# giech/usrp_nfc

Measured on AMD Instinct MI355X. Metric: IQ Msamples/s -> decoded bits (2 Msps stream), higher is better.
Workload: dtype f32 envelope / f64 window sums / u8 symbols; 1 GPU; configs[1]: Miller-only decode, synthetic IQ @2 Msps; input_kind=fc32 IQ, 8 B/sample (envelope computed in the kernel), samples_per_gpu=100000000, parallelism=time-chunk x1, edges_per_gpu=6627699, symbols_reader=3971547, symbols_tag=0, packets=101186, boundary_redos=0, exchange=none, stepping=sync, in_flight=1

## Files before the change

### usrp_nfc_amd/csrc/host_context.h

```cpp
#pragma once


namespace {

std::string g_create_error;

}

enum : int {
    TOT_RUNS = 0,
    TOT_EDGES = 8,
    TOT_DECMAP = 16,
    TOT_SPEC = 40,
    TOT_PKT0 = 72,
    TOT_PKT1 = 80,
    TOT_LAST2 = 88,
    TOT_NSYM = 96,
    TOT_CERT = 104,
    TOT_FRAME = 128,
    TOT_BYTES = 160
};

static_assert(sizeof(CertSummary) <= TOT_FRAME - TOT_CERT, "the verdict summary fits its slot of the totals");
struct DevState {
// ... 1 lines not shown
    EdgeCarry ecarry;
    DecCarry dcarry;
    uint8_t totals[TOT_BYTES];
    uint32_t seq[4];
};

constexpr size_t AHEAD_LDS_MAX = 96 * 1024;
constexpr int LEAN_STEPS_AHEAD = 4;
constexpr int NRING = 4;
constexpr int NSUB = 3;

namespace {
struct Switches {
    std::optional<std::string> debug_clk;
    std::optional<int> no_small, debug_bad_launch, debug_redo_submitted, debug, trace, trace_alloc, no_submit_ahead, wg, wg_rounds, wg_bulk, wg_rerun, wg_rowbal, wg_nr, wg_per_cu, wg_per_cu_ahead, wg_ex, lean, lean_rounds,
        lean_waves, edge_prefix, dec_spec, dec_runin, spin_wait, chunk_adapt, chunk_mult;
    std::optional<double> lean_gfac, lean_gmin, eps;
    std::optional<unsigned long> own_prefix_max;
    std::optional<std::pair<int, int>> wg_lone;
    std::optional<std::array<double, 3>> rowbal_f;
    std::optional<bool> ring_global;
};
inline Switches read_switches() {
    Switches s;
#ifdef NFC_TEST_HOOKS
    const struct { const char *name; std::optional<int> Switches::*at; } ints[] = {
        {"NFC_NO_SMALL", &Switches::no_small}, {"NFC_DEBUG_BAD_LAUNCH", &Switches::debug_bad_launch}, {"NFC_DEBUG_REDO_SUBMITTED", &Switches::debug_redo_submitted},
        {"NFC_DEBUG", &Switches::debug}, {"NFC_TRACE", &Switches::trace}, {"NFC_TRACE_ALLOC", &Switches::trace_alloc}, {"NFC_NO_SUBMIT_AHEAD", &Switches::no_submit_ahead},
        {"NFC_WG", &Switches::wg}, {"NFC_WG_ROUNDS", &Switches::wg_rounds}, {"NFC_WG_BULK", &Switches::wg_bulk},
        {"NFC_WG_RERUN", &Switches::wg_rerun}, {"NFC_WG_NR", &Switches::wg_nr}, {"NFC_WG_PER_CU", &Switches::wg_per_cu},
        {"NFC_WG_PER_CU_AHEAD", &Switches::wg_per_cu_ahead}, {"NFC_WG_EX", &Switches::wg_ex}, {"NFC_LEAN", &Switches::lean}, {"NFC_LEAN_ROUNDS", &Switches::lean_rounds},
        {"NFC_LEAN_WAVES", &Switches::lean_waves}, {"NFC_EDGE_PREFIX", &Switches::edge_prefix}, {"NFC_DEC_SPEC", &Switches::dec_spec}, {"NFC_DEC_RUNIN", &Switches::dec_runin},
        {"NFC_SPIN_WAIT", &Switches::spin_wait}, {"NFC_CHUNK_ADAPT", &Switches::chunk_adapt}, {"NFC_CHUNK_MULT", &Switches::chunk_mult}};
    const struct { const char *name; std::optional<double> Switches::*at; } reals[] = {
        {"NFC_LEAN_GFAC", &Switches::lean_gfac}, {"NFC_LEAN_GMIN", &Switches::lean_gmin}, {"NFC_EPS", &Switches::eps}};
    for (const auto &v : ints)
        if (const char *e = getenv(v.name)) s.*v.at = atoi(e);
    for (const auto &v : reals)
        if (const char *e = getenv(v.name)) s.*v.at = atof(e);
    if (const char *e = getenv("NFC_DEBUG_CLK")) s.debug_clk = e;
    if (const char *e = getenv("NFC_OWN_PREFIX_MAX")) s.own_prefix_max = strtoul(e, nullptr, 10);
    if (const char *e = getenv("NFC_WG_LONE")) {
        int a = 4, b = 64;
        if (sscanf(e, "%d,%d", &a, &b) >= 1) s.wg_lone = std::make_pair(a, b);
    }
    if (const char *e = getenv("NFC_WG_ROWBAL")) {
        std::array<double, 3> f{0.0, 1.0, 1.0};
        if (sscanf(e, "%lf,%lf,%lf", &f[0], &f[1], &f[2]) >= 2 && f[0] > 0.5 && f[0] < 1.5 && f[1] > 0.5 && f[1] < 1.5 && f[2] > 0.5 && f[2] < 1.5)
// ... 48 lines not shown
    float eps;
    float i16_scale;
    size_t in_bytes_per_sample;
    hipStream_t st = nullptr;
    Stream own_st;
    Stream st_a;
    Event ev[8];
    DevBuf d_gring;
    bool state_dirty = false, dirty_fill_ring = false;
    float dirty_fill = 0.f;
    Carry dirty_carry;
    EdgeCarry dirty_ecarry;
    DecCarry dirty_dcarry;
    bool cert_pending = false;
    CertLaunch cert;
    bool dbg_bad_launch = false, dbg_redo_submitted = false, dbg_no_submit_ahead = false, dbg_any = false, dbg_clk = false, dbg_trace = false;
    std::string dbg_clk_path;
    uint32_t batch_seq = 0;
    int timing = 0;
    Event kev[2 * 6];
    int n_kev = 0;
    std::string err;
    LaunchError launch_err;

    DevBuf d_mil_map, d_man_map, d_mil_out, d_man_out, d_qmil_map, d_qmil_step;
    uint8_t mil_q_of[16], mil_canon[16];
    DecTables T;

    DevBuf d_state, d_ring[NRING];
    PinBuf hs_pin{hipHostMallocMapped | hipHostMallocCoherent};
// ... 156 lines not shown
    LaunchError &le = launch_error();
    if (le.err != hipSuccess) {
        const LaunchError e = le;
        le = LaunchError{};
        return fail(c, NFC_ERR_DEVICE, "kernel launch failed: %s (%s:%d)", hipGetErrorString(e.err), e.file, e.line);
    }
    if (with_mirror && c->hs->seq[0] != c->batch_seq)
        return fail(c, NFC_ERR_DEVICE, "state mirror is stale (batch %u, mirror %u): a kernel of this batch did not run", c->batch_seq, c->hs->seq[0]);
    return NFC_OK;
}
#define BATCHCHK(c, with_mirror)                                   \
    do {                                                           \
        if (int rc__ = batch_ok((c), (with_mirror))) return rc__;  \
    } while (0)

void launch_fill_kind(nfc_ctx *c, const void *in, uint32_t n, int nchunks, int ring_idx = -1) {
    float *ring = c->d_ring[ring_idx < 0 ? c->ring_cur : ring_idx].as<float>();
    Carry *cr = dC(c);
    EdgeCarryInit eci{(int32_t *)dE(c), c->L % c->mx};
    uint8_t *ver = c->d_ver.as<uint8_t>();
    CertSummary *sum = (CertSummary *)(dT(c) + TOT_CERT);
    StateInit init;
    memset(&init, 0, sizeof init);
    int fresh = 0;
    if (c->state_dirty) {
        static_assert(offsetof(DevState, totals) <= sizeof init.words && offsetof(DevState, totals) % 4 == 0, "state head fits");
        DevState h;
        h.carry = c->dirty_carry;
        h.ecarry = c->dirty_ecarry;
        h.dcarry = c->dirty_dcarry;
        init.apply = 1;
        init.n_words = (int32_t)(offsetof(DevState, totals) / 4);
        memcpy(init.words, &h, offsetof(DevState, totals));
        init.dst = (uint32_t *)c->d_state.p;
        init.fill_ring = c->dirty_fill_ring ? 1 : 0;
        init.fill = c->dirty_fill;
        init.ring_len = c->Lpad;
        c->state_dirty = c->dirty_fill_ring = false;
        fresh = h.carry.stable == 0 && h.carry.filled == 0 && n >= (uint32_t)c->L && (void *)cr == c->d_state.p;
    }
    NFC_LAUNCH(c->kk->fill, dim3(1), dim3(FILL_BLOCK), (size_t)c->Lpad * 4, c->st, in, n, c->i16_scale, c->L, ring, cr, eci, ver, nchunks, sum, init,
               &((DevState *)c->d_state.p)->seq[0], c->batch_seq, fresh);
}
void launch_seq_kind(nfc_ctx *c, const SeqArgs &A) { NFC_LAUNCH(c->kk->seq, dim3(1), dim3(64), 0, c->st, A); }

int ceil_log2(int v) {
    int b = 0;
    while ((1 << b) < v) b++;
    return b;
}

double elapsed_ms(hipEvent_t a, hipEvent_t b) {
    float ms = 0;
    (void)hipEventElapsedTime(&ms, a, b);
    return ms;
}

// ... 3 lines not shown
```

### usrp_nfc_amd/csrc/host_stages.h

```cpp
#pragma once

namespace {

__global__ __launch_bounds__(256) void k_certify_and_write(CertLaunch C, EdgeArgs E, size_t nwords, const EdgeAgg *partials, const EdgeAgg *supers,
                                                          const EdgeRec *recs, uint32_t *epos, uint16_t *ecode, uint32_t cap, bool own_prefix, uint32_t *total_out,
                                                          Last2 *last2_total, EdgeCarry *carry_out) {
    const uint32_t tiles = gridDim.x - C.blocks;
    if (blockIdx.x == 0) {
        certify_block(C.A, C.cert, nullptr, C.ring_next, C.carry, C.sum, C.blocks - 1, C.blocks);
        return;
    }
    if (blockIdx.x > tiles) {
        certify_block(C.A, C.cert, nullptr, C.ring_next, C.carry, C.sum, blockIdx.x - tiles - 1, C.blocks);
        return;
    }
    write_edges_tile(E, nwords, partials, supers, recs, epos, ecode, cap, own_prefix, total_out, last2_total, carry_out, tiles - blockIdx.x, tiles);
}

int run_edges(nfc_ctx *c, uint32_t n, uint32_t skip, uint64_t g0, bool beside_threshold = false) {
    uint8_t *tot = dT(c);
    const size_t nwords = ((size_t)n + 63) / 64;
    EdgeArgs E;
    E.neg = c->d_neg.as<uint64_t>();
    E.pos = c->d_pos.as<uint64_t>();
    E.n = n;
    E.skip = skip;
    E.mx = c->mx;
    E.dur_in = c->h_ecarry.dur;
    E.last_bit_in = c->h_ecarry.last_bit;
    E.state_in = c->h_ecarry.state;
    E.nd = c->mx + 1;
// ... 3 lines not shown
    for (int b = 0; b < 64; b += c->mx) E.per_mask |= 1ull << b;
    E.sw = (uint32_t)(EW_WORDS * EW_SUPER);
    E.tps = (uint32_t)EW_SUPER;
    const size_t tiles = edge_num_tiles(nwords);
    const size_t supers = edge_num_supers(nwords);
    HIPCHK(c, c->d_partials.ensure((tiles + supers + 2) * sizeof(EdgeAgg)));
    EdgeAgg *parts = c->d_partials.as<EdgeAgg>();
    EdgeAgg *sups = parts + tiles + 1;
    const bool use_recs = c->edge_prefix < 0 ? !beside_threshold : c->edge_prefix != 0;
    if (use_recs) HIPCHK(c, c->d_edge_rec.ensure(std::max<size_t>(tiles, 1) * SCAN_BLOCK * sizeof(EdgeRec)));
    EdgeRec *recs = use_recs ? c->d_edge_rec.as<EdgeRec>() : nullptr;
    const bool own = tiles <= c->own_prefix_max;
    Last2 *last2_total = (Last2 *)(tot + TOT_LAST2);
    uint32_t *edges_total = (uint32_t *)(tot + TOT_EDGES);
    const EdgeAggOp op{E.mx, E.mx_magic};
    if (tiles) NFC_LAUNCH(k_edge_reduce, dim3((unsigned)supers), dim3(ER_BLOCK), 0, c->st, E, nwords, parts, sups, recs);
    if (!own || !tiles)
        scan_partials_with(c->st, op, supers, nullptr, (uint32_t)(EW_WORDS * EW_SUPER), sups, op.identity(), (EdgeAgg *)nullptr,
                           EdgeTotalEpilogue{E, edges_total, last2_total, dE(c)});
    const uint32_t cap = c->cap_edges;
    const size_t cap_al = std::max(cap, c->alloc_edges);
    HIPCHK(c, c->d_epos.ensure((cap_al + 8) * 4));
    HIPCHK(c, c->d_ecode.ensure((cap_al + 8) * 2));
    if (c->cert_pending && tiles) {
        c->cert_pending = false;
        NFC_LAUNCH(k_certify_and_write, dim3((unsigned)(c->cert.blocks + tiles)), dim3(SCAN_BLOCK), 0, c->st, c->cert, E, nwords, parts, sups, recs,
                   c->d_epos.as<uint32_t>(), c->d_ecode.as<uint16_t>(), cap, own, edges_total, last2_total, dE(c));
    } else if (tiles) {
        NFC_LAUNCH(k_write_edges, dim3((unsigned)tiles), dim3(SCAN_BLOCK), 0, c->st, E, nwords, parts, sups, recs, c->d_epos.as<uint32_t>(),
                   c->d_ecode.as<uint16_t>(), cap, own, edges_total, last2_total, dE(c));
    }
// ... 349 lines not shown
            }
            const int r = run_small(c, n, skip, g0);
            if (r) return r;
            if (!ev3_done && c->timing >= 2) HIPCHK(c, hipEventRecord(c->ev[3], c->st));
            ev3_done = true;
            return NFC_OK;
        }
        int r = run_edges(c, n, skip, g0);
        if (r) return r;
        if (!ev3_done && c->timing >= 2) HIPCHK(c, hipEventRecord(c->ev[3], c->st));
        ev3_done = true;
        return run_decode(c);
    };
    const std::function<int()> ahead = edges_and_decode;
    bool clean = false;
    int rc = run_threshold(c, d_in, n, skip, want_edges ? &ahead : nullptr, &clean);
    if (rc) return rc;
    if (want_edges) {
        bool decode_only = false;
        int respeculated = 0;
        for (int attempt = 0;; attempt++) {
            if (attempt > 0 || !clean || decode_only) {
                if (decode_only) {
                    rc = run_decode(c, true);
                } else {
                    rc = edges_and_decode();
                }
                if (rc) return rc;
                HIPCHK(c, hipStreamSynchronize(c->st));
            }
// ... 73 lines not shown
```

### usrp_nfc_amd/csrc/host_threshold.h

```cpp
#pragma once

namespace {

static bool sums_exact(const Carry &hc, int emin, int emax, uint32_t vtop) {
    int low = emin - 23;
    if (hc.ss_emin != 255) low = std::min(low, hc.ss_emin);
    float vtf;
    memcpy(&vtf, &vtop, 4);
    int high = 255 + 64;
    if (std::isfinite(vtf) && vtf >= 0.f) high = vtf > 0.f ? std::ilogb((double)vtf) + 127 : 0;
    high = std::max(high, hc.ss_emax);
    return (emax < 255) && (high - low <= 52);
}

static inline void eps_adapt(nfc_ctx *c, const CertSummary &s) {
    if (!c->dbg_trace) return;
    float w;
    memcpy(&w, &s.worst, 4);
    fprintf(stderr, "[nfc] eps %.5f: the speculation used %.5f of the window sum at most, %u chunks failed their certification\n", (double)c->eps, (double)w, s.n_fail);
}

static inline void cpu_relax() {
#if defined(__x86_64__) || defined(__i386__)
    __builtin_ia32_pause();
// ... 244 lines not shown
    A.nlist = 0;
    A.mode = 0;
    A.cert = P.d_cert;
    A.sum = (CertSummary *)(dT(c) + TOT_CERT);
    A.ksteps = P.form == ThrForm::Workgroup ? c->wg_rounds : c->lean_rounds;
    A.gfac = c->lean_gfac;
    A.gfloor = c->lean_gmin;
    A.blk = 1 << c->nfold;
    launch_threshold(c, P, ThrLaunch::Pass0, A, P.nch, own_events);
}
static void enqueue_certify(nfc_ctx *c, const ThrPlan &P, const ThrArgs &A, CertInfo *info, float *ring_out, CertSummary *sum) {
    NFC_LAUNCH(k_certify, dim3(cert_grid(A.nlist)), dim3(256), 0, c->st, A, P.d_cert, info, ring_out, dC(c), sum);
}

static int threshold_span(nfc_ctx *c, const void *d_in_all, uint32_t n_all, uint32_t skip_all, uint32_t base, const EdgeCarry &ec,
                          const std::function<int()> *ahead, bool *clean, bool *need_seq_out, bool *recut_out = nullptr) {
    bool ran_ahead = false;
    *clean = false;
    const int L = c->L;
    const uint32_t n = n_all - base;
    const uint32_t skip = skip_all > base ? skip_all - base : 0u;
    const void *d_in = (const char *)d_in_all + (size_t)base * c->in_bytes_per_sample;
    const uint64_t nseen = c->nseen + base;
    uint32_t passes = 0;
    ThrArgs A;
    ThrPlan P;
    if (int rc = thr_prepare(c, d_in, n, n_all, skip, base, nseen, ec, c->ring_cur, c->d_neg, c->d_pos, false, A, P)) return rc;
    const uint32_t nch = P.nch;
    const bool wg = P.form == ThrForm::Workgroup;
    uint8_t *d_cert = P.d_cert;
    const uint8_t *h_cert = P.h_cert, *h_gflags = P.h_gflags, *h_gmin = P.h_gmin, *h_gmax = P.h_gmax;

    launch_fill_kind(c, d_in, n, (int)nch);

    const bool force_seq = (c->P.flags & NFC_FLAG_FORCE_SEQUENTIAL) != 0 || L < STEP;
    bool need_seq = force_seq;
    if (!force_seq) {
        const bool lean = wg || P.form == ThrForm::Lean;
        const bool dbg_clk = lean && c->dbg_clk;
        if (dbg_clk) {
            HIPCHK(c, c->d_certinfo.ensure((size_t)nch * 32 * 5));
            A.dbg_clk = c->d_certinfo.as<unsigned long long>();
        }
        enqueue_pass0(c, P, A);
        if (dbg_clk) {
            std::vector<unsigned long long> h((size_t)nch * 4);
            HIPCHK(c, hipStreamSynchronize(c->st));
            HIPCHK(c, hipMemcpy(h.data(), c->d_certinfo.p, (size_t)nch * 32, hipMemcpyDeviceToHost));
            unsigned long long t0 = ~0ull, t1 = 0;
            double pro = 0, loop = 0, epi = 0, maxtot = 0, maxstart = 0;
            for (uint32_t k = 0; k < nch; k++) {
                t0 = std::min(t0, h[4 * k]);
                t1 = std::max(t1, h[4 * k + 3]);
            }
            for (uint32_t k = 0; k < nch; k++) {
                pro += (double)(h[4 * k + 1] - h[4 * k]);
                loop += (double)(h[4 * k + 2] - h[4 * k + 1]);
                epi += (double)(h[4 * k + 3] - h[4 * k + 2]);
                maxtot = std::max(maxtot, (double)(h[4 * k + 3] - h[4 * k]));
// ... 78 lines not shown
                flags_with_verdict = first_round && c->fine_left > 0;
                if (!first_round || flags_with_verdict) {
                    HIPCHK(c, hipMemcpyAsync(c->h_cflags.p, c->d_cflags.p, (size_t)4 * nch, hipMemcpyDeviceToHost, c->st));
                    HIPCHK(c, hipMemcpyAsync(P.h_gvtop, c->d_gvtop.p, (size_t)nch * 4, hipMemcpyDeviceToHost, c->st));
                }
                HIPCHK(c, mirror_async(c));
                if (first_round && ahead) {
                    const int rc = (*ahead)();
                    if (rc) return rc;
                    ran_ahead = true;
                }
            }
            if (stamped_last) HIPCHK(c, wait_for_stamp(c));
            else HIPCHK(c, hipStreamSynchronize(c->st));
            BATCHCHK(c, true);
            std::vector<uint32_t> failing;
            if (first_round) {
                memcpy(&summary, c->hs->totals + TOT_CERT, sizeof summary);
                if (base == 0) eps_adapt(c, summary);
                if (summary.n_fail == 0 && !dbg) {
                    have_summary = true;
                    break;
                }
                if (recut_out && c->fine_adapt && wg && c->fine_left == 0 && !c->P.chunk_samples && c->fine_mult > 1 &&
                    (uint64_t)summary.n_fail * 64u > (uint64_t)nch) {
                    *recut_out = true;
                    A.ver_zero = 0;
                    return NFC_OK;
                }
                if (!flags_with_verdict) HIPCHK(c, hipMemcpy(c->h_cflags.p, c->d_cflags.p, (size_t)4 * nch, hipMemcpyDeviceToHost));
// ... 189 lines not shown
    return NFC_OK;
}

int run_threshold(nfc_ctx *c, const void *d_in, uint32_t n, uint32_t skip, const std::function<int()> *ahead, bool *clean) {
    *clean = false;
    c->stats.threshold_passes = 0;
    c->stats.chunks_rerun = 0;
    c->stats.chunks_rerun_in_place = 0;
    c->stats.used_sequential = 0;
    const uint32_t span = (uint32_t)std::min<uint64_t>(((uint64_t)8 * c->L + STEP - 1) / STEP * STEP, 1u << 30);
    EdgeCarry ec = c->h_ecarry;
    uint32_t base = 0;
    for (int round = 0;; round++) {
        bool need_seq = false, span_clean = false;
        const bool optimistic = base == 0 && !(c->fine_adapt && c->fine_left > 0);
        bool recut = false;
        int rc = threshold_span(c, d_in, n, skip, base, ec, optimistic ? ahead : nullptr, &span_clean, &need_seq, &recut);
        if (rc) return rc;
        if (recut) {
            c->fine_left = 8;
            c->cert_pending = false;
            HIPCHK(c, hipMemsetAsync((char *)dC(c) + offsetof(Carry, fin_valid), 0, sizeof(int32_t), c->st));
            span_clean = false;
            rc = threshold_span(c, d_in, n, skip, base, ec, nullptr, &span_clean, &need_seq, nullptr);
            if (rc) return rc;
        }
        if (!need_seq) {
            *clean = span_clean && base == 0;
            if (c->fine_adapt) {
                if ((uint64_t)c->stats.chunks_rerun * 64u > (uint64_t)c->stats.n_chunks) c->fine_left = 8;
                else if (c->fine_left > 0) c->fine_left--;
            }
            return NFC_OK;
        }
        const bool forced = (c->P.flags & NFC_FLAG_FORCE_SEQUENTIAL) != 0 || c->L < STEP;
// ... 11 lines not shown
```

### usrp_nfc_amd/csrc/nfc_amd.hip

```cpp
#include <hip/hip_runtime.h>
#include <hip/hip_ext.h>

#include <algorithm>
#include <atomic>
#include <chrono>
#include <cmath>
#include <cstdarg>
#include <cstdio>
#include <cstdlib>
#include <cstring>
#include <string>
#include <thread>
#include <array>
#include <functional>
#include <memory>
#include <optional>
#include <vector>

#include "../../include/nfc_amd.h"
#include "launch_check.h"
#include "decode.hip.h"
#include "decoder_tables.h"
#include "edges.hip.h"
#include "scan.hip.h"
// ... 183 lines not shown
    if (c->wg_ex_ok) {
        const void *kx = (const void *)c->kk->wg_ex;
        if (c->wg_ex_lds > 64 * 1024) CRT(hipFuncSetAttribute(kx, hipFuncAttributeMaxDynamicSharedMemorySize, (int)c->wg_ex_lds));
        int fit = 0;
        CRT(hipOccupancyMaxActiveBlocksPerMultiprocessor(&fit, kx, 256, c->wg_ex_lds));
        if (fit < 1) c->wg_ex_ok = 0;
        c->wg_ex_max = prop.multiProcessorCount * std::max(1, std::min(4, fit));
    }
    if (sw.wg_ex) {
        if (*sw.wg_ex <= 0) c->wg_ex_ok = 0;
        else c->wg_ex_max = *sw.wg_ex;
    }
    if (!c->wg_rounds) c->wg_rounds = 8;
    if (sw.chunk_adapt) c->fine_adapt = *sw.chunk_adapt != 0;
    if (sw.chunk_mult) c->fine_mult = std::max(1, std::min(16, *sw.chunk_mult));
    return NFC_OK;
}

int create_resources(nfc_ctx *c) {
    CRT(c->own_st.create());
    c->st = c->own_st;
    for (auto &e : c->ev) CRT(e.create());
    for (auto &e : c->kev) CRT(e.create());
    CRT(c->st_a.create());
    for (int b = 0; b < NSUB; b++) {
        CRT(c->ev_a[b].create(hipEventDisableTiming));
        CRT(c->ev_b[b].create(hipEventDisableTiming));
        CRT(c->kev_sub[b][0].create());
        CRT(c->kev_sub[b][1].create());
        CRT(c->hs_a[b].ensure(sizeof(DevState)));
// ... 1063 lines not shown
#ifdef NFC_TEST_HOOKS
extern "C" float nfc_debug_frames_ms(const nfc_ctx *c) { return c && c->frames_ready ? c->fr_ms : -1.f; }
extern "C" void nfc_debug_live_resources(uint64_t out[4]) {
    for (int k = 0; k < 4; k++) out[k] = nfc::live::count(k).load();
}
extern "C" int nfc_debug_dec_lds(const nfc_ctx *c, int which, uint32_t *dyn_bytes, int *wgs_per_cu) {
    if (!c || which < 0 || which > 2 || !dyn_bytes || !wgs_per_cu) return NFC_ERR_ARG;
    const bool lds = 4 * c->T.nd <= nfc::DEC_LDS_ROWS;
    const void *k = which == 0   ? (const void *)nfc::dec_spec_kernel(lds, c->T)
                    : which == 1 ? (lds ? (const void *)nfc::k_dec_reduce<true> : (const void *)nfc::k_dec_reduce<false>)
                                 : (lds ? (const void *)nfc::k_dec_apply<true> : (const void *)nfc::k_dec_apply<false>);
    *dyn_bytes = (uint32_t)c->dec_lds[which];
    if (hipSetDevice(c->P.device) != hipSuccess) return NFC_ERR_DEVICE;
    return hipOccupancyMaxActiveBlocksPerMultiprocessor(wgs_per_cu, k, nfc::SCAN_BLOCK, c->dec_lds[which]) == hipSuccess ? NFC_OK : NFC_ERR_DEVICE;
}
extern "C" int nfc_debug_dec_shapes(const nfc_ctx *c, uint32_t *out6) {
    if (!c || !out6) return NFC_ERR_ARG;
    out6[0] = (uint32_t)nfc::DEC_TILE;
    out6[1] = c->own_prefix_max;
    out6[2] = nfc::ST_CLOSES;
    out6[3] = (uint32_t)nfc::DEC_LDS_ROWS;
    out6[4] = (uint32_t)(nfc::DEC_RUNIN_MAX * nfc::SCAN_BLOCK);
    out6[5] = c->sym_own ? 1u : 0u;
    return NFC_OK;
}
#endif
```

### usrp_nfc_amd/csrc/threshold.hip.h

```cpp
#pragma once
#include <hip/hip_runtime.h>
#include <stdint.h>

#include <type_traits>

namespace nfc {

constexpr int STEP = 256;
constexpr int LL_NONE = -(1 << 30);
constexpr int MAX_FIX_ITERS = 80;
constexpr float RND_SUM = 2.44140625e-04f;

enum : int { IN_IQ_F32 = 0, IN_ENV_F32 = 1, IN_REAL_F32_SQ = 2, IN_I16_SQ = 3, IN_IQ_I16 = 4, IN_IQ_I8 = 5, IN_IQ_U8 = 6 };

#ifndef NFC_HDR_KERNEL_LINKAGE
#define NFC_HDR_KERNEL_LINKAGE
#endif

struct Carry {
    double ss;
    double delta;
    int32_t filled;
    int32_t stable;
    int32_t ss_emin;
// ... 66 lines not shown
    uint32_t nlist;
    int32_t mode;
    int32_t twords;
    int32_t off;
    int32_t nrows;
    uint8_t *cert;
    CertSummary *sum;
    int32_t ksteps;
    float gfac, gfloor;
    int32_t blk;
    int32_t ver_zero;
    int32_t wg_stage_rounds;
    unsigned long long *dbg_clk;
    uint32_t row_len[4], row_start[4], row_div;
    int C_max;
};
__device__ __forceinline__ void chunk_span(const ThrArgs &A, uint32_t c, uint32_t &m_chunk, uint32_t &len) {
    const uint32_t row = min(c / A.row_div, 3u);
    len = A.row_len[row];
    m_chunk = A.row_start[row] + (c - row * A.row_div) * len;
}

__device__ __forceinline__ int rfl(int v) { return __builtin_amdgcn_readfirstlane(v); }
__device__ __forceinline__ uint32_t rfl(uint32_t v) { return (uint32_t)__builtin_amdgcn_readfirstlane((int)v); }
__device__ __forceinline__ float rfl(float v) { return __int_as_float(__builtin_amdgcn_readfirstlane(__float_as_int(v))); }
__device__ __forceinline__ double rfl(double v) {
    return __hiloint2double(__builtin_amdgcn_readfirstlane(__double2hiint(v)), __builtin_amdgcn_readfirstlane(__double2loint(v)));
}
__device__ __forceinline__ bool uni(bool c) { return __builtin_amdgcn_readfirstlane((int)c) != 0; }
template <int CTRL, int ROWMASK>
// ... 1153 lines not shown
    }
}

struct EdgeCarryInit {
    int32_t *dst;
    int32_t dur0;
};

struct StateInit {
    int32_t apply, fill_ring, ring_len, n_words;
    float fill;
    uint32_t *dst;
    uint32_t words[32];
};

template <int KIND>
__global__ __launch_bounds__(FILL_BLOCK) void k_fill(const void *in, uint32_t n, float i16_scale, int L, float *ring, Carry *carry,
                                                     EdgeCarryInit eci, uint8_t *ver, int nchunks, CertSummary *sum, StateInit init,
                                                     uint32_t *seq_dst, uint32_t seq, int fresh) {
    extern __shared__ __attribute__((aligned(16))) unsigned char smem[];
    __shared__ FillRed red;
    float *lr = (float *)smem;
    const int tid = threadIdx.x;
    if (tid == 0 && seq_dst) *seq_dst = seq;
    if (fresh) {
        static_assert(sizeof(Carry) % 4 == 0 && sizeof(Carry) <= sizeof(init.words), "the carry heads the state block");
        constexpr int CW = (int)(sizeof(Carry) / 4);
        if (tid >= CW && tid < init.n_words) init.dst[tid] = init.words[tid];
        double part = 0;
        uint32_t emin = 255u, emax = 0u;
// ... 7 lines not shown
                if (i >= L) break;
                ring[i] = v[k];
                lr[i] = v[k];
                part += (double)v[k];
                if (v[k] != 0.f) {
                    const uint32_t e = max(f32_expfield(v[k]), 1u);
                    emin = min(emin, e);
                    emax = max(emax, e);
                }
            }
        }
        if (init.fill_ring)
            for (int i = L + tid; i < init.ring_len; i += FILL_BLOCK) ring[i] = 0.f;
        for (int i = tid; i < nchunks; i += FILL_BLOCK) ver[i] = 0;
        fill_reduce(red, part, emin, emax);
        if (tid == 0) {
            const double S = part;
            int lg = 0;
            while ((1 << lg) < L) lg++;
            const bool exact = (emax < 255u) && ((int)emax + 2 + lg - ((int)emin - 23) <= 52);
            double s = S, err = 0;
            if (!exact) {
                s = 0;
                for (int i = 0; i < L; i++) {
                    const double v = (double)lr[i];
                    const double t = s + v;
                    const double bv = t - s;
                    err += fabs((s - (t - bv)) + (v - bv));
                    s = t;
                }
            }
            Carry nc;
            uint32_t cw[CW];
#pragma unroll
            for (int k = 0; k < CW; k++) cw[k] = init.words[k];
            memcpy(&nc, cw, sizeof nc);
            nc.filled = L;
            nc.ss = s;
            nc.stable = 1;
            if (err != 0.0) nc.inexact = 1;
            batch_guard(nc, S, emin, emax);
            *carry = nc;
            eci.dst[0] = 0;
            eci.dst[1] = 0;
            eci.dst[2] = eci.dur0;
            if (sum) *sum = CertSummary{0u, 255u, 0u, 0u, 0u, 0u};
        }
        return;
    }
    if (init.apply) {
        if (tid < init.n_words) init.dst[tid] = init.words[tid];
        if (init.fill_ring)
            for (int i = tid; i < init.ring_len; i += FILL_BLOCK) ring[i] = i < L ? init.fill : 0.f;
        __syncthreads();
    }
    if (carry->stable) {
        prepare_batch(ring, L, carry, ver, nchunks, sum, red);
        return;
    }
    const int filled = carry->filled;
    const int can = min((int)n, L - filled);
    double part = 0;
// ... 38 lines not shown
                const double bv = t - s;
                err += fabs((s - (t - bv)) + (v - bv));
                s = t;
            }
        }
        carry->filled = L;
        carry->ss = s;
        carry->stable = 1;
        if (err != 0.0) carry->inexact = 1;
        eci.dst[0] = 0;
        eci.dst[1] = 0;
        eci.dst[2] = eci.dur0;
    }
    for (int i = tid; i < nchunks; i += FILL_BLOCK) ver[i] = 0;
    prepare_batch_finish(carry, sum, S, emin, emax);
}

NFC_HDR_KERNEL_LINKAGE __global__ __launch_bounds__(FIN_BLOCK) void k_finalize_state(ThrArgs A, float *ring_next, Carry *carry) {
    finalize_state(A, ring_next, carry, nullptr);
}

struct SeqArgs {
    const void *in;
    uint32_t n, skip, g0modL;
    int32_t L, mx;
    double lo, hi, hi_plus;
    float i16_scale;
    float *ring;
    Carry *carry;
    int32_t state, last_bit, dur;
// ... 56 lines not shown
```

### usrp_nfc_amd/csrc/threshold_wg.hip.h

```cpp
#pragma once
#include "edges.hip.h"
#include "threshold_lean.hip.h"

namespace nfc {

constexpr int WG_WAVES = 4;
constexpr int wg_round_samples(int nr) { return 64 * nr * WG_WAVES; }
constexpr int WG_NR_MAX = 8;
#ifndef NFC_WG_FR
#define NFC_WG_FR 8
#endif
constexpr int wg_flush_rounds(int nr) { return nr == 4 ? NFC_WG_FR : NFC_WG_FR / 2; }
constexpr size_t wg_stage_bytes(int nr, int rounds) { return (size_t)rounds * (size_t)(2 * WG_WAVES * 2 * nr * 4); }
struct WgShared {
    uint32_t msk[3][WG_WAVES][4 * WG_NR_MAX + 4];
    uint32_t scr[2][WG_WAVES][8];
    int32_t fin[WG_WAVES][4];
    float4 acc[WG_WAVES][64];
    uint32_t flag[WG_WAVES];
    uint32_t cold[WG_WAVES][8];
    float bc[8];
};
constexpr size_t WG_SHARED_BYTES = (sizeof(WgShared) + 15) & ~(size_t)15;

// ... 150 lines not shown
    const int mx = A.mx;
    uint32_t m_chunk_v, chunk_len_v;
    chunk_span(A, c, m_chunk_v, chunk_len_v);
    const uint32_t m_chunk = rfl(m_chunk_v), chunk_len = rfl(chunk_len_v);
    const uint32_t n1 = min(A.n, m_chunk + chunk_len);
    const uint32_t m_start = max(m_chunk, A.skip);
    constexpr int RB = LeanRaw<KIND>::BYTES;
    const uint32_t wbase0 = m_chunk + STEPN * (uint32_t)wave;
    const char *const in_first = (const char *)A.in + (size_t)wbase0 * RB;
    const uint32_t voff = (uint32_t)lane * (uint32_t)RB;
    bool primed = false;
    if (m_chunk >= m_start && m_chunk + (uint32_t)wg_round_samples(NR) <= n1) {
        wg_load_step<KIND, NR>(voff, in_first);
        primed = true;
    }
    const Carry cr = *A.carry;
    uint64_t *const neg_p = A.neg, *const pos_p = A.pos;
    const uintptr_t plane_of_lane = (lane >= 2 * NR) ? (uintptr_t)pos_p : (uintptr_t)neg_p;
    const int plane_dword = (lane >= 2 * NR) ? lane - 2 * NR : lane;
    const float i16s = A.i16_scale;
    const unsigned long long lane_lt = (1ull << lane) - 1ull;
    int scr_par = 0;
    auto wg_gather = [&](const uint32_t (&v)[8], int k, uint32_t (&out)[WG_WAVES][8]) __attribute__((always_inline)) {
        if (lane == 0)
            for (int i = 0; i < k; i++) sh->scr[scr_par][wave][i] = v[i];
        wg_barrier();
        for (int w = 0; w < WG_WAVES; w++)
            for (int i = 0; i < k; i++) out[w][i] = rfl(sh->scr[scr_par][w][i]);
        scr_par ^= 1;
    };

// ... 20 lines not shown
#ifdef NFC_WG_PROF
    unsigned long long pf_take = 0, pf_b1 = 0, pf_b2 = 0, pf_rounds = 0, pf_t = 0;
#define WG_PF_BEGIN() pf_t = clock64()
#define WG_PF_END(acc) acc += clock64() - pf_t
#else
#define WG_PF_BEGIN() ((void)0)
#define WG_PF_END(acc) ((void)0)
#endif
    if (A.dbg_clk) clk0 = clock64();

    uint32_t emin = 255u, emax = 0u, vtop0 = 0u;
    int nl_in, kl_in;
    float ssf, eps = 0.f;
    {
        double ss0;
        if (c == 0) {
            for (int s = tid; s < L; s += 256) ring[s] = A.ring_carry[s];
            ss0 = cr.ss;
            nl_in = carried_nl(A);
            kl_in = carried_kl(A);
            wg_barrier();
        } else if (A.mode == 1) {
            double part = 0;
            for (int s = tid; s < L; s += 256) {
                const float v = resolve_slot(A, (int)c, s);
                ring[s] = v;
                part += (double)v;
            }
            const double ps = wave_sum_f64(part);
            uint32_t v[8], g[WG_WAVES][8];
            v[0] = (uint32_t)__double2loint(ps);
// ... 98 lines not shown
        uint32_t v[8], g[WG_WAVES][8];
        v[0] = wave_max_u32(vtop0);
        v[1] = wave_min_u32(emin);
        v[2] = wave_max_u32(emax);
        wg_gather(v, 3, g);
        vtop0 = max(max(g[0][0], g[1][0]), max(g[2][0], g[3][0]));
        emin = min(min(g[0][1], g[1][1]), min(g[2][1], g[3][1]));
        emax = max(max(g[0][2], g[1][2]), max(g[2][2], g[3][2]));
    }
    nl_in = rfl(nl_in);
    kl_in = rfl(kl_in);

    if (A.dbg_clk) clk1 = clock64();
    bool good_run = A.fast_ok != 0;
    if constexpr (KIND == IN_ENV_F32) good_run = good_run && vtop0 < 0x7F800000u;
    uint32_t why = good_run ? 0u : 1u;
    float min_ss = 3.0e38f;
    uint32_t vmin = 0xFFFFFFFFu, vmax = vtop0;
    const float etaD = 1.0f - 9.5367431640625e-07f;
    const float slU = 1.0f + 3.814697265625e-06f;
    const float loLf = (float)A.lo_L, hiLf = (float)A.hi_L;
    uint32_t slot_step = (A.g0modL + wbase0) % (uint32_t)L;
    const uint32_t slot_adv = (uint32_t)WG_ROUND % (uint32_t)L;
    float b_acc = 0.f, dl_acc = 0.f;
    float tlo = 0.f, thi = 0.f;
    float dlo = 3.0e38f, dhi = 3.0e38f;
    uint32_t xlo_acc = 0x7F7FFFFFu, xhi_acc = 0u;
    int lz_base = LL_NONE;
    int rounds_since_sync = 0;
    float xkeep[NR], snap[NR];
// ... 843 lines not shown
    }

#ifdef NFC_EX_PRINTF
    if (EX && tid == 0) printf("chunk %u: %d of %d rounds exact (codes %x, first %d last %d, %d trips) good %d why %u; cycles: prologue %llu rounds %llu (in place %llu) summary-so-far %llu\n", c, ex_count, n_rounds, ex_codes, ex_first, ex_last, ex_trips, (int)good_run, why, ex_t1 - ex_t0, ex_ta - ex_t1, ex_tx, clock64() - ex_ta);
#endif
    if (A.dbg_clk) clk2 = clock64();
    const uint32_t all_robust = good_run ? 1u : 0u;
    if (c == 0 && tid == 0 && A.mode == 0) {
        A.cert[0] = good_run ? 1 : 0;
        if (!good_run) atomicAdd(&A.sum->n_fail, 1u);
    }
    {
        uint32_t v[8], g[WG_WAVES][8];
        v[0] = min(wave_min_u32(vmin), rfl(sh->cold[wave][2]));
        v[1] = max(wave_max_u32(vmax), rfl(sh->cold[wave][3]));
        const int vb_new = (A.mode == 1) ? 1 - (int)A.ver[c] : (int)A.ver[c];
        float *ro = (vb_new ? A.ring_out[1] : A.ring_out[0]) + (size_t)c * L;
        uint32_t *to = (vb_new ? A.touched[1] : A.touched[0]) + (size_t)c * A.twords;
        uint32_t untouched = 0;
        for (int sbase = 64 * wave; sbase < A.twords * 32; sbase += 256) {
            const int s = sbase + lane;
            const float rv = (s < L) ? ring[s] : 0.f;
            const bool t = (s < L) && !(__float_as_uint(rv) >> 31);
            const unsigned long long bal = __ballot(t);
            if (s < L) {
                __builtin_nontemporal_store(fabsf(rv), ro + s);
                if (!t) untouched++;
            }
            const int w = sbase >> 5;
            if (lane == 0) {
                to[w] = (uint32_t)bal;
// ... 57 lines not shown
```

Measured before the change: 447,900 Msamples/s.

## Defer fresh window fill into edge-reduce launch and let pass 0 build its own window

On a fresh stream the separate single-workgroup fill kernel no longer runs ahead of pass 0. Chunk 0 of pass 0 now computes the initial window envelope itself, assuming a zero delta passed by value. The fill's carry, certificate and summary work rides as an extra workgroup of the later edge-reduce launch. This is meant to take a serial one-block kernel off the critical path before the threshold pass. If the carried delta turns out nonzero, the span is redone in the original order, which adds host bookkeeping and a fallback path.

```diff
diff --git a/usrp_nfc_amd/csrc/host_context.h b/usrp_nfc_amd/csrc/host_context.h
--- a/usrp_nfc_amd/csrc/host_context.h
+++ b/usrp_nfc_amd/csrc/host_context.h
@@ -39,7 +39,7 @@
 struct Switches {
     std::optional<std::string> debug_clk;
     std::optional<int> no_small, debug_bad_launch, debug_redo_submitted, debug, trace, trace_alloc, no_submit_ahead, wg, wg_rounds, wg_bulk, wg_rerun, wg_rowbal, wg_nr, wg_per_cu, wg_per_cu_ahead, wg_ex, lean, lean_rounds,
-        lean_waves, edge_prefix, dec_spec, dec_runin, spin_wait, chunk_adapt, chunk_mult;
+        lean_waves, edge_prefix, dec_spec, dec_runin, spin_wait, chunk_adapt, chunk_mult, fill_front;
     std::optional<double> lean_gfac, lean_gmin, eps;
     std::optional<unsigned long> own_prefix_max;
     std::optional<std::pair<int, int>> wg_lone;
@@ -56,7 +56,7 @@
         {"NFC_WG_RERUN", &Switches::wg_rerun}, {"NFC_WG_NR", &Switches::wg_nr}, {"NFC_WG_PER_CU", &Switches::wg_per_cu},
         {"NFC_WG_PER_CU_AHEAD", &Switches::wg_per_cu_ahead}, {"NFC_WG_EX", &Switches::wg_ex}, {"NFC_LEAN", &Switches::lean}, {"NFC_LEAN_ROUNDS", &Switches::lean_rounds},
         {"NFC_LEAN_WAVES", &Switches::lean_waves}, {"NFC_EDGE_PREFIX", &Switches::edge_prefix}, {"NFC_DEC_SPEC", &Switches::dec_spec}, {"NFC_DEC_RUNIN", &Switches::dec_runin},
-        {"NFC_SPIN_WAIT", &Switches::spin_wait}, {"NFC_CHUNK_ADAPT", &Switches::chunk_adapt}, {"NFC_CHUNK_MULT", &Switches::chunk_mult}};
+        {"NFC_SPIN_WAIT", &Switches::spin_wait}, {"NFC_CHUNK_ADAPT", &Switches::chunk_adapt}, {"NFC_CHUNK_MULT", &Switches::chunk_mult}, {"NFC_FILL_FRONT", &Switches::fill_front}};
     const struct { const char *name; std::optional<double> Switches::*at; } reals[] = {
         {"NFC_LEAN_GFAC", &Switches::lean_gfac}, {"NFC_LEAN_GMIN", &Switches::lean_gmin}, {"NFC_EPS", &Switches::eps}};
     for (const auto &v : ints)
@@ -135,6 +135,9 @@
     DecCarry dirty_dcarry;
     bool cert_pending = false;
     CertLaunch cert;
+    bool fill_pending = false, fill_can_ride = false, fill_front = false;
+    FillRider fill;
+    uint32_t dbg_fill_rode = 0, dbg_fill_refront = 0;
     bool dbg_bad_launch = false, dbg_redo_submitted = false, dbg_no_submit_ahead = false, dbg_any = false, dbg_clk = false, dbg_trace = false;
     std::string dbg_clk_path;
     uint32_t batch_seq = 0;
@@ -321,7 +324,7 @@
         if (int rc__ = batch_ok((c), (with_mirror))) return rc__;  \
     } while (0)
 
-void launch_fill_kind(nfc_ctx *c, const void *in, uint32_t n, int nchunks, int ring_idx = -1) {
+bool launch_fill_kind(nfc_ctx *c, const void *in, uint32_t n, int nchunks, int ring_idx = -1, const uint8_t *ride_cert0 = nullptr) {
     float *ring = c->d_ring[ring_idx < 0 ? c->ring_cur : ring_idx].as<float>();
     Carry *cr = dC(c);
     EdgeCarryInit eci{(int32_t *)dE(c), c->L % c->mx};
@@ -346,8 +349,15 @@
         c->state_dirty = c->dirty_fill_ring = false;
         fresh = h.carry.stable == 0 && h.carry.filled == 0 && n >= (uint32_t)c->L && (void *)cr == c->d_state.p;
     }
+    uint32_t *const seq_dst = &((DevState *)c->d_state.p)->seq[0];
+    if (fresh && ride_cert0) {
+        c->fill = FillRider{c->L, nchunks, ring, cr, eci, ver, ride_cert0, sum, seq_dst, c->batch_seq, init};
+        c->fill_pending = true;
+        return true;
+    }
     NFC_LAUNCH(c->kk->fill, dim3(1), dim3(FILL_BLOCK), (size_t)c->Lpad * 4, c->st, in, n, c->i16_scale, c->L, ring, cr, eci, ver, nchunks, sum, init,
-               &((DevState *)c->d_state.p)->seq[0], c->batch_seq, fresh);
+               seq_dst, c->batch_seq, fresh);
+    return false;
 }
 void launch_seq_kind(nfc_ctx *c, const SeqArgs &A) { NFC_LAUNCH(c->kk->seq, dim3(1), dim3(64), 0, c->st, A); }
 
diff --git a/usrp_nfc_amd/csrc/host_stages.h b/usrp_nfc_amd/csrc/host_stages.h
--- a/usrp_nfc_amd/csrc/host_stages.h
+++ b/usrp_nfc_amd/csrc/host_stages.h
@@ -15,6 +15,15 @@
         return;
     }
     write_edges_tile(E, nwords, partials, supers, recs, epos, ecode, cap, own_prefix, total_out, last2_total, carry_out, tiles - blockIdx.x, tiles);
+}
+
+static_assert(ER_BLOCK == FILL_BLOCK, "the rider is one workgroup of the reduce pass");
+__global__ __launch_bounds__(ER_BLOCK) void k_edge_reduce_and_fill(FillRider F, EdgeArgs E, size_t nwords, EdgeAgg *partials, EdgeAgg *supers, EdgeRec *recs) {
+    if (blockIdx.x == 0) {
+        fill_rider(F);
+        return;
+    }
+    edge_reduce_super(E, nwords, blockIdx.x - 1, partials, supers, recs);
 }
 
 int run_edges(nfc_ctx *c, uint32_t n, uint32_t skip, uint64_t g0, bool beside_threshold = false) {
@@ -48,7 +57,12 @@
     Last2 *last2_total = (Last2 *)(tot + TOT_LAST2);
     uint32_t *edges_total = (uint32_t *)(tot + TOT_EDGES);
     const EdgeAggOp op{E.mx, E.mx_magic};
-    if (tiles) NFC_LAUNCH(k_edge_reduce, dim3((unsigned)supers), dim3(ER_BLOCK), 0, c->st, E, nwords, parts, sups, recs);
+    if (tiles && c->fill_pending) {
+        c->fill_pending = false;
+        NFC_LAUNCH(k_edge_reduce_and_fill, dim3((unsigned)supers + 1u), dim3(ER_BLOCK), 0, c->st, c->fill, E, nwords, parts, sups, recs);
+    } else if (tiles) {
+        NFC_LAUNCH(k_edge_reduce, dim3((unsigned)supers), dim3(ER_BLOCK), 0, c->st, E, nwords, parts, sups, recs);
+    }
     if (!own || !tiles)
         scan_partials_with(c->st, op, supers, nullptr, (uint32_t)(EW_WORDS * EW_SUPER), sups, op.identity(), (EdgeAgg *)nullptr,
                            EdgeTotalEpilogue{E, edges_total, last2_total, dE(c)});
@@ -428,6 +442,8 @@
     };
     const std::function<int()> ahead = edges_and_decode;
     bool clean = false;
+    c->fill_pending = false;
+    c->fill_can_ride = want_edges && !(c->use_small && n <= SM_MAX_SAMPLES);
     int rc = run_threshold(c, d_in, n, skip, want_edges ? &ahead : nullptr, &clean);
     if (rc) return rc;
     if (want_edges) {
diff --git a/usrp_nfc_amd/csrc/host_threshold.h b/usrp_nfc_amd/csrc/host_threshold.h
--- a/usrp_nfc_amd/csrc/host_threshold.h
+++ b/usrp_nfc_amd/csrc/host_threshold.h
@@ -282,7 +282,8 @@
 }
 
 static int threshold_span(nfc_ctx *c, const void *d_in_all, uint32_t n_all, uint32_t skip_all, uint32_t base, const EdgeCarry &ec,
-                          const std::function<int()> *ahead, bool *clean, bool *need_seq_out, bool *recut_out = nullptr) {
+                          const std::function<int()> *ahead, bool *clean, bool *need_seq_out, bool *recut_out = nullptr,
+                          bool *refront_out = nullptr) {
     bool ran_ahead = false;
     *clean = false;
     const int L = c->L;
@@ -299,9 +300,9 @@
     uint8_t *d_cert = P.d_cert;
     const uint8_t *h_cert = P.h_cert, *h_gflags = P.h_gflags, *h_gmin = P.h_gmin, *h_gmax = P.h_gmax;
 
-    launch_fill_kind(c, d_in, n, (int)nch);
-
     const bool force_seq = (c->P.flags & NFC_FLAG_FORCE_SEQUENTIAL) != 0 || L < STEP;
+    const bool may_ride = wg && !force_seq && ahead && !c->dbg_any && c->fill_can_ride && !c->fill_front && refront_out;
+    const bool rode = launch_fill_kind(c, d_in, n, (int)nch, -1, may_ride ? P.d_cert : nullptr);
     bool need_seq = force_seq;
     if (!force_seq) {
         const bool lean = wg || P.form == ThrForm::Lean;
@@ -310,7 +311,10 @@
             HIPCHK(c, c->d_certinfo.ensure((size_t)nch * 32 * 5));
             A.dbg_clk = c->d_certinfo.as<unsigned long long>();
         }
+        A.delta_by_value = A.own_window = rode ? 1 : 0;
+        A.delta_val = 0.0;
         enqueue_pass0(c, P, A);
+        A.delta_by_value = A.own_window = 0;
         if (dbg_clk) {
             std::vector<unsigned long long> h((size_t)nch * 4);
             HIPCHK(c, hipStreamSynchronize(c->st));
@@ -419,6 +423,16 @@
             if (stamped_last) HIPCHK(c, wait_for_stamp(c));
             else HIPCHK(c, hipStreamSynchronize(c->st));
             BATCHCHK(c, true);
+            if (first_round && rode) {
+                if (c->fill_pending) return fail(c, NFC_ERR_INTERNAL, "the window fill was left behind pass 0 and no launch took it");
+                c->dbg_fill_rode++;
+                if (!(c->hs->carry.delta == 0.0)) {
+                    c->dbg_fill_refront++;
+                    *refront_out = true;
+                    A.ver_zero = 0;
+                    return NFC_OK;
+                }
+            }
             std::vector<uint32_t> failing;
             if (first_round) {
                 memcpy(&summary, c->hs->totals + TOT_CERT, sizeof summary);
@@ -638,11 +652,11 @@
     for (int round = 0;; round++) {
         bool need_seq = false, span_clean = false;
         const bool optimistic = base == 0 && !(c->fine_adapt && c->fine_left > 0);
-        bool recut = false;
-        int rc = threshold_span(c, d_in, n, skip, base, ec, optimistic ? ahead : nullptr, &span_clean, &need_seq, &recut);
+        bool recut = false, refront = false;
+        int rc = threshold_span(c, d_in, n, skip, base, ec, optimistic ? ahead : nullptr, &span_clean, &need_seq, &recut, &refront);
         if (rc) return rc;
-        if (recut) {
-            c->fine_left = 8;
+        if (recut || refront) {
+            if (recut) c->fine_left = 8;
             c->cert_pending = false;
             HIPCHK(c, hipMemsetAsync((char *)dC(c) + offsetof(Carry, fin_valid), 0, sizeof(int32_t), c->st));
             span_clean = false;
diff --git a/usrp_nfc_amd/csrc/nfc_amd.hip b/usrp_nfc_amd/csrc/nfc_amd.hip
--- a/usrp_nfc_amd/csrc/nfc_amd.hip
+++ b/usrp_nfc_amd/csrc/nfc_amd.hip
@@ -221,6 +221,7 @@
     if (!c->wg_rounds) c->wg_rounds = 8;
     if (sw.chunk_adapt) c->fine_adapt = *sw.chunk_adapt != 0;
     if (sw.chunk_mult) c->fine_mult = std::max(1, std::min(16, *sw.chunk_mult));
+    if (sw.fill_front) c->fill_front = *sw.fill_front != 0;
     return NFC_OK;
 }
 
@@ -1314,6 +1315,12 @@
     if (hipSetDevice(c->P.device) != hipSuccess) return NFC_ERR_DEVICE;
     return hipOccupancyMaxActiveBlocksPerMultiprocessor(wgs_per_cu, k, nfc::SCAN_BLOCK, c->dec_lds[which]) == hipSuccess ? NFC_OK : NFC_ERR_DEVICE;
 }
+extern "C" int nfc_debug_fill_order(const nfc_ctx *c, uint32_t *out2) {
+    if (!c || !out2) return NFC_ERR_ARG;
+    out2[0] = c->dbg_fill_rode;
+    out2[1] = c->dbg_fill_refront;
+    return NFC_OK;
+}
 extern "C" int nfc_debug_dec_shapes(const nfc_ctx *c, uint32_t *out6) {
     if (!c || !out6) return NFC_ERR_ARG;
     out6[0] = (uint32_t)nfc::DEC_TILE;
diff --git a/usrp_nfc_amd/csrc/threshold.hip.h b/usrp_nfc_amd/csrc/threshold.hip.h
--- a/usrp_nfc_amd/csrc/threshold.hip.h
+++ b/usrp_nfc_amd/csrc/threshold.hip.h
@@ -104,6 +104,9 @@
     unsigned long long *dbg_clk;
     uint32_t row_len[4], row_start[4], row_div;
     int C_max;
+    double delta_val;
+    int32_t delta_by_value;
+    int32_t own_window;
 };
 __device__ __forceinline__ void chunk_span(const ThrArgs &A, uint32_t c, uint32_t &m_chunk, uint32_t &len) {
     const uint32_t row = min(c / A.row_div, 3u);
@@ -1287,6 +1290,40 @@
     uint32_t words[32];
 };
 
+__device__ __forceinline__ void fresh_finish(const StateInit &init, int L, const float *win, double S, uint32_t emin, uint32_t emax, Carry *carry,
+                                             EdgeCarryInit eci, CertSummary *sum, uint32_t n_fail0) {
+    constexpr int CW = (int)(sizeof(Carry) / 4);
+    int lg = 0;
+    while ((1 << lg) < L) lg++;
+    const bool exact = (emax < 255u) && ((int)emax + 2 + lg - ((int)emin - 23) <= 52);
+    double s = S, err = 0;
+    if (!exact) {
+        s = 0;
+        for (int i = 0; i < L; i++) {
+            const double v = (double)win[i];
+            const double t = s + v;
+            const double bv = t - s;
+            err += fabs((s - (t - bv)) + (v - bv));
+            s = t;
+        }
+    }
+    Carry nc;
+    uint32_t cw[CW];
+#pragma unroll
+    for (int k = 0; k < CW; k++) cw[k] = init.words[k];
+    memcpy(&nc, cw, sizeof nc);
+    nc.filled = L;
+    nc.ss = s;
+    nc.stable = 1;
+    if (err != 0.0) nc.inexact = 1;
+    batch_guard(nc, S, emin, emax);
+    *carry = nc;
+    eci.dst[0] = 0;
+    eci.dst[1] = 0;
+    eci.dst[2] = eci.dur0;
+    if (sum) *sum = CertSummary{n_fail0, 255u, 0u, 0u, 0u, 0u};
+}
+
 template <int KIND>
 __global__ __launch_bounds__(FILL_BLOCK) void k_fill(const void *in, uint32_t n, float i16_scale, int L, float *ring, Carry *carry,
                                                      EdgeCarryInit eci, uint8_t *ver, int nchunks, CertSummary *sum, StateInit init,
@@ -1324,38 +1361,7 @@
             for (int i = L + tid; i < init.ring_len; i += FILL_BLOCK) ring[i] = 0.f;
         for (int i = tid; i < nchunks; i += FILL_BLOCK) ver[i] = 0;
         fill_reduce(red, part, emin, emax);
-        if (tid == 0) {
-            const double S = part;
-            int lg = 0;
-            while ((1 << lg) < L) lg++;
-            const bool exact = (emax < 255u) && ((int)emax + 2 + lg - ((int)emin - 23) <= 52);
-            double s = S, err = 0;
-            if (!exact) {
-                s = 0;
-                for (int i = 0; i < L; i++) {
-                    const double v = (double)lr[i];
-                    const double t = s + v;
-                    const double bv = t - s;
-                    err += fabs((s - (t - bv)) + (v - bv));
-                    s = t;
-                }
-            }
-            Carry nc;
-            uint32_t cw[CW];
-#pragma unroll
-            for (int k = 0; k < CW; k++) cw[k] = init.words[k];
-            memcpy(&nc, cw, sizeof nc);
-            nc.filled = L;
-            nc.ss = s;
-            nc.stable = 1;
-            if (err != 0.0) nc.inexact = 1;
-            batch_guard(nc, S, emin, emax);
-            *carry = nc;
-            eci.dst[0] = 0;
-            eci.dst[1] = 0;
-            eci.dst[2] = eci.dur0;
-            if (sum) *sum = CertSummary{0u, 255u, 0u, 0u, 0u, 0u};
-        }
+        if (tid == 0) fresh_finish(init, L, lr, part, emin, emax, carry, eci, sum, 0u);
         return;
     }
     if (init.apply) {
@@ -1424,6 +1430,42 @@
     }
     for (int i = tid; i < nchunks; i += FILL_BLOCK) ver[i] = 0;
     prepare_batch_finish(carry, sum, S, emin, emax);
+}
+
+struct FillRider {
+    int32_t L, nchunks;
+    float *ring;
+    Carry *carry;
+    EdgeCarryInit eci;
+    uint8_t *ver;
+    const uint8_t *cert0;
+    CertSummary *sum;
+    uint32_t *seq_dst;
+    uint32_t seq;
+    StateInit init;
+};
+__device__ __forceinline__ void fill_rider(const FillRider &F) {
+    __shared__ FillRed red;
+    constexpr int CW = (int)(sizeof(Carry) / 4);
+    const int tid = threadIdx.x;
+    if (tid == 0) *F.seq_dst = F.seq;
+    if (tid >= CW && tid < F.init.n_words) F.init.dst[tid] = F.init.words[tid];
+    double part = 0;
+    uint32_t emin = 255u, emax = 0u;
+    for (int i = tid; i < F.L; i += FILL_BLOCK) {
+        const float v = F.ring[i];
+        part += (double)v;
+        if (v != 0.f) {
+            const uint32_t e = max(f32_expfield(v), 1u);
+            emin = min(emin, e);
+            emax = max(emax, e);
+        }
+    }
+    if (F.init.fill_ring)
+        for (int i = F.L + tid; i < F.init.ring_len; i += FILL_BLOCK) F.ring[i] = 0.f;
+    for (int i = tid; i < F.nchunks; i += FILL_BLOCK) F.ver[i] = 0;
+    fill_reduce(red, part, emin, emax);
+    if (tid == 0) fresh_finish(F.init, F.L, F.ring, part, emin, emax, F.carry, F.eci, F.sum, *F.cert0 ? 0u : 1u);
 }
 
 NFC_HDR_KERNEL_LINKAGE __global__ __launch_bounds__(FIN_BLOCK) void k_finalize_state(ThrArgs A, float *ring_next, Carry *carry) {
diff --git a/usrp_nfc_amd/csrc/threshold_wg.hip.h b/usrp_nfc_amd/csrc/threshold_wg.hip.h
--- a/usrp_nfc_amd/csrc/threshold_wg.hip.h
+++ b/usrp_nfc_amd/csrc/threshold_wg.hip.h
@@ -188,7 +188,14 @@
         wg_load_step<KIND, NR>(voff, in_first);
         primed = true;
     }
-    const Carry cr = *A.carry;
+    struct { double ss, delta; } cr;
+    if (A.delta_by_value) {
+        cr.ss = 0.0;
+        cr.delta = A.delta_val;
+    } else {
+        cr.ss = A.carry->ss;
+        cr.delta = A.carry->delta;
+    }
     uint64_t *const neg_p = A.neg, *const pos_p = A.pos;
     const uintptr_t plane_of_lane = (lane >= 2 * NR) ? (uintptr_t)pos_p : (uintptr_t)neg_p;
     const int plane_dword = (lane >= 2 * NR) ? lane - 2 * NR : lane;
@@ -239,7 +246,37 @@
     float ssf, eps = 0.f;
     {
         double ss0;
-        if (c == 0) {
+        if (c == 0 && A.own_window) {
+            float *const rc = const_cast<float *>(A.ring_carry);
+            double part = 0;
+            for (int i0 = 0; i0 < L; i0 += 2048) {
+                typename RawOf<KIND>::T rw[8];
+#pragma unroll
+                for (int k = 0; k < 8; k++) {
+                    const int i = i0 + 256 * k + tid;
+                    rw[k] = (i < L) ? load_raw<KIND>(A.in, (size_t)i) : raw_zero<KIND>();
+                }
+#pragma unroll
+                for (int k = 0; k < 8; k++) {
+                    const int i = i0 + 256 * k + tid;
+                    if (i < L) {
+                        const float x = env_of<KIND>(rw[k], A.i16_scale);
+                        ring[i] = x;
+                        rc[i] = x;
+                        part += (double)x;
+                    }
+                }
+            }
+            const double ps = wave_sum_f64(part);
+            uint32_t v[8], g[WG_WAVES][8];
+            v[0] = (uint32_t)__double2loint(ps);
+            v[1] = (uint32_t)__double2hiint(ps);
+            wg_gather(v, 2, g);
+            ss0 = 0;
+            for (int w = 0; w < WG_WAVES; w++) ss0 += __hiloint2double((int)g[w][1], (int)g[w][0]);
+            nl_in = carried_nl(A);
+            kl_in = carried_kl(A);
+        } else if (c == 0) {
             for (int s = tid; s < L; s += 256) ring[s] = A.ring_carry[s];
             ss0 = cr.ss;
             nl_in = carried_nl(A);
@@ -368,6 +405,11 @@
     if (A.dbg_clk) clk1 = clock64();
     bool good_run = A.fast_ok != 0;
     if constexpr (KIND == IN_ENV_F32) good_run = good_run && vtop0 < 0x7F800000u;
+    if (c == 0 && A.own_window) {
+        int lg = 0;
+        while ((1 << lg) < L) lg++;
+        good_run = good_run && emax < 255u && (int)emax + 2 + lg - ((int)emin - 23) <= 52;
+    }
     uint32_t why = good_run ? 0u : 1u;
     float min_ss = 3.0e38f;
     uint32_t vmin = 0xFFFFFFFFu, vmax = vtop0;
@@ -1241,7 +1283,7 @@
         uint32_t v[8], g[WG_WAVES][8];
         v[0] = min(wave_min_u32(vmin), rfl(sh->cold[wave][2]));
         v[1] = max(wave_max_u32(vmax), rfl(sh->cold[wave][3]));
-        const int vb_new = (A.mode == 1) ? 1 - (int)A.ver[c] : (int)A.ver[c];
+        const int vb_new = A.delta_by_value ? 0 : (A.mode == 1) ? 1 - (int)A.ver[c] : (int)A.ver[c];
         float *ro = (vb_new ? A.ring_out[1] : A.ring_out[0]) + (size_t)c * L;
         uint32_t *to = (vb_new ? A.touched[1] : A.touched[0]) + (size_t)c * A.twords;
         uint32_t untouched = 0;
```

Result: faster. 458,100 Msamples/s (median of 6 runs) (+2.3%).
